# jeffpeterson/hypermerge

Hardware: AMD Instinct MI355X
Metric: merged changes/sec (1M docs×8 actors) at 1/2/4/8 GPUs + % HBM roofline (higher is better)
Workload: dtype u32; 1 GPU; C4: 1000000 docs/GPU x 8 actors x 64 changes/doc, map LWW sets; docs_per_gpu=1000000, changes_per_gpu=64000000, ops_per_gpu=96000538, parallelism=doc-shard1

## Files before the change

hypermerge_amd/csrc/merge_kernels.hip:

```cpp
#include <hip/hip_runtime.h>
#include <stdint.h>
#include "../../include/hypermerge_amd.h"
#include "merge_kernels.h"
#include "wave.h"

#ifndef HM_ABLATE
#define HM_ABLATE 0
#endif
#ifndef HM_STAMPS
#define HM_STAMPS 0
#endif
#define HM_NSTAMP 20
#ifndef HM_WAVES_PER_EU_OPL4
#define HM_WAVES_PER_EU_OPL4 3
#endif
#ifndef HM_WAVES_PER_EU_LIST3
#define HM_WAVES_PER_EU_LIST3 3
#endif
#ifndef HM_PRIO_PUSH
#define HM_PRIO_PUSH 2
#endif
#ifndef HM_PRIO_IO
#define HM_PRIO_IO 1
#endif
#ifndef HM_PRIO_HIST
#define HM_PRIO_HIST 3
#endif
#ifndef HM_PRIO_RANK
#define HM_PRIO_RANK 2
#endif
#ifndef HM_PRIO_K2
#define HM_PRIO_K2 2
#endif
#ifndef HM_PRIO_K1
#define HM_PRIO_K1 3
#endif
#ifndef HM_ASYNC_MAX_OPL
#define HM_ASYNC_MAX_OPL 2
#endif
#ifndef HM_ASYNC_STORES
#define HM_ASYNC_STORES 10
#endif
#ifndef HM_ASYNC_CHECK
#define HM_ASYNC_CHECK 0
#endif
#ifndef HM_WAVES_PER_EU
#define HM_WAVES_PER_EU 5
#endif
#ifndef HM_WAVES_PER_EU_WIDE
#define HM_WAVES_PER_EU_WIDE 4
#endif
#define WAVE 64
#define NA_MAX 8
#define NDEP_MAX 1024
typedef unsigned long long u64;
#if defined(__HIP_DEVICE_COMPILE__)
#define LDS __attribute__((address_space(3)))
#else
#define LDS
#endif

namespace hm {

__device__ __forceinline__ u64 readlane64(u64 v, int l) {
    const uint32_t lo = __builtin_amdgcn_readlane((int)(uint32_t)v, l);
    const uint32_t hi = __builtin_amdgcn_readlane((int)(uint32_t)(v >> 32), l);
    return ((u64)hi << 32) | lo;
}
__device__ __forceinline__ uint32_t shfl32(uint32_t v, int src) {
    return (uint32_t)__builtin_amdgcn_ds_bpermute(src << 2, (int)v);
}
__device__ __forceinline__ u64 shfl64(u64 v, int src) {
    return ((u64)shfl32((uint32_t)(v >> 32), src) << 32) | shfl32((uint32_t)v, src);
}
__device__ __forceinline__ u64 wave_or64(u64 v) {
    for (int o = 1; o < WAVE; o <<= 1) v |= shfl64(v, (int)(threadIdx.x ^ o));
    return v;
}
__device__ __forceinline__ uint32_t wave_excl_scan(uint32_t v, uint32_t *total) {
    uint32_t x = v;
    x += (uint32_t)__builtin_amdgcn_update_dpp(0, (int)x, DPP_ROW_SHR(1), 0xF, 0xF, false);
    x += (uint32_t)__builtin_amdgcn_update_dpp(0, (int)x, DPP_ROW_SHR(2), 0xF, 0xF, false);
    x += (uint32_t)__builtin_amdgcn_update_dpp(0, (int)x, DPP_ROW_SHR(4), 0xF, 0xF, false);
    x += (uint32_t)__builtin_amdgcn_update_dpp(0, (int)x, DPP_ROW_SHR(8), 0xF, 0xF, false);
    x += (uint32_t)__builtin_amdgcn_update_dpp(0, (int)x, DPP_ROW_BCAST15, 0xA, 0xF, false);
    x += (uint32_t)__builtin_amdgcn_update_dpp(0, (int)x, DPP_ROW_BCAST31, 0xC, 0xF, false);
    *total = (uint32_t)__builtin_amdgcn_readlane((int)x, WAVE - 1);
    return x - v;
}
__device__ __forceinline__ uint32_t wave_max(uint32_t v) {
    uint32_t x = v, y;
    y = (uint32_t)__builtin_amdgcn_update_dpp(0, (int)x, DPP_ROW_SHR(1), 0xF, 0xF, false); x = x > y ? x : y;
    y = (uint32_t)__builtin_amdgcn_update_dpp(0, (int)x, DPP_ROW_SHR(2), 0xF, 0xF, false); x = x > y ? x : y;
    y = (uint32_t)__builtin_amdgcn_update_dpp(0, (int)x, DPP_ROW_SHR(4), 0xF, 0xF, false); x = x > y ? x : y;
    y = (uint32_t)__builtin_amdgcn_update_dpp(0, (int)x, DPP_ROW_SHR(8), 0xF, 0xF, false); x = x > y ? x : y;
    y = (uint32_t)__builtin_amdgcn_update_dpp(0, (int)x, DPP_ROW_BCAST15, 0xA, 0xF, false); x = x > y ? x : y;
    y = (uint32_t)__builtin_amdgcn_update_dpp(0, (int)x, DPP_ROW_BCAST31, 0xC, 0xF, false); x = x > y ? x : y;
    return (uint32_t)__builtin_amdgcn_readlane((int)x, WAVE - 1);
}
__device__ __forceinline__ uint32_t bytesum64(u64 x) {
    return __builtin_amdgcn_sad_u8((uint32_t)x, 0u, __builtin_amdgcn_sad_u8((uint32_t)(x >> 32), 0u, 0u));
}
__device__ __forceinline__ uint32_t prev_lane(uint32_t v) {
    return (uint32_t)__builtin_amdgcn_update_dpp(0, (int)v, DPP_WAVE_SHR1, 0xF, 0xF, false);
}
__device__ __forceinline__ uint32_t fresh_lane() {
    uint32_t l;
    asm volatile("v_mov_b32 %0, %1" : "=v"(l) : "v"((uint32_t)threadIdx.x));
    return l;
}
template <bool FRESH> __device__ __forceinline__ uint32_t lane_id() {
    if constexpr (FRESH) return fresh_lane();
    else return threadIdx.x;
}
template <int OPL, bool LISTS, int CLS> struct Diet { static constexpr bool on = OPL <= 2 && !LISTS && CLS != 1; };
__device__ __forceinline__ void wave_sync() {
    __builtin_amdgcn_fence(__ATOMIC_SEQ_CST, "wavefront");
    __builtin_amdgcn_wave_barrier();
}

__device__ __forceinline__ u64 err_key(uint32_t h, uint32_t op_plus1, uint32_t arr, uint32_t code) {
    return ((u64)h << 40) | ((u64)(op_plus1 & 0xFFFF) << 24) | ((u64)(arr & 0xFFFF) << 8) | code;
}

struct SmallLds {
    LDS u64 *anc, *chain, *segor, *errkey, *cov;
    LDS u64 *opval;
    LDS u64 *survpk;
    LDS int64_t *survsum;
    LDS uint32_t *first, *base, *bclock, *headv, *objslot, *segcnt, *survcnt, *regoff, *regobj, *insmin;
    LDS uint32_t *flags, *deps, *depinfo;
    LDS uint8_t *seglist;
    LDS uint16_t *survp;
    LDS uint32_t *opro;
    LDS uint32_t *opmeta;
    LDS uint32_t *opelem;
    LDS int32_t *hist_of;
    LDS uint16_t *survop, *opbase;
    LDS uint16_t *oppar;
    LDS uint8_t *h2a, *chactor, *objtype;
    LDS uint16_t *opchg;
    LDS uint32_t *nins, *pcount, *nodekey, *tour0, *listbase;
    LDS uint16_t *poff;
    LDS uint16_t *nodeop, *nodepi, *regnode, *plist, *fc, *ns, *listid;
    LDS u64 *stamps;
};
#define PAR_HEAD 0xFFFFu
template <bool LISTS> struct Stride {
    static constexpr uint32_t reg = LISTS ? 1 : 4;
    static constexpr uint32_t seg = LISTS ? 1 : 2;
    static constexpr uint32_t op = LISTS ? 1 : 2;
};

template <int CLS> struct SizeClass;
template <> struct SizeClass<0> { static constexpr uint32_t NR = 32, NO = 16, ND = 128; };
template <> struct SizeClass<1> { static constexpr uint32_t NR = 256, NO = 64, ND = 512; };
template <> struct SizeClass<2> { static constexpr uint32_t NR = 128, NO = 32, ND = 256; };

template <typename L_t, typename P>
__host__ __device__ inline size_t small_carve(P base, uint32_t NOp, uint32_t NR, uint32_t NO, uint32_t ND,
                                              bool lists, bool counters, L_t *L) {
    size_t o = 0;
#define TAKE(f, T, cnt) do { L->f = (decltype(L->f))(base + o); o = (o + (size_t)(cnt) * sizeof(T) + 15) & ~(size_t)15; } while (0)
    TAKE(anc, u64, 64);          TAKE(chain, u64, NA_MAX);     TAKE(opval, u64, NOp);
    TAKE(errkey, u64, 1);        TAKE(base, uint32_t, NA_MAX * 3);
    if (lists) {
        TAKE(survcnt, uint32_t, NR); TAKE(regoff, uint32_t, NR);   TAKE(regobj, uint32_t, NR);
        TAKE(insmin, uint32_t, NR);  TAKE(flags, uint32_t, 2);
        TAKE(opmeta, uint32_t, NOp); TAKE(opro, uint32_t, NOp);
    } else {
        TAKE(survcnt, uint32_t, 4 * NR);                           TAKE(flags, uint32_t, 2);
        L->regoff = L->survcnt + 1; L->insmin = L->survcnt + 2;    L->regobj = L->survcnt + 3;
        TAKE(opro, uint32_t, 2 * NOp);
        L->opmeta = L->opro + 1;
    }
    TAKE(survop, uint16_t, NOp); TAKE(chactor, uint8_t, 64);   TAKE(objtype, uint8_t, NO);
    if (lists) {
        TAKE(opelem, uint32_t, NOp);
        L->nodekey = L->opelem;
        TAKE(nins, uint32_t, 1);
    }
    TAKE(stamps, u64, HM_STAMPS ? HM_NSTAMP + 1 : 0);
    const size_t dead_at = o;
    TAKE(hist_of, int32_t, 64);  TAKE(cov, u64, 1);            TAKE(opbase, uint16_t, 64);
    TAKE(oppar, uint16_t, lists ? NOp : 0);
    TAKE(h2a, uint8_t, 64);      TAKE(opchg, uint16_t, NOp);
    const size_t k1_at = o;
    TAKE(first, uint32_t, NA_MAX * 64);
    TAKE(deps, uint32_t, ND > NOp ? ND : NOp);
    TAKE(depinfo, uint32_t, ND);
    const size_t k1_end = o;
    o = k1_at;
    if (lists) { TAKE(segor, u64, NR);  TAKE(survpk, u64, NR); }
    else { TAKE(segor, u64, 2 * NR);    L->survpk = L->segor + 1; }
    TAKE(segcnt, uint32_t, NR);
    TAKE(objslot, uint32_t, NO);
    if (o < k1_end) o = k1_end;
    L->seglist = (decltype(L->seglist))L->first; L->survp = (decltype(L->survp))L->first;
    if (lists) {
        const uint32_t NP = NR + NO, NE = 2 * (NOp + NO);
        size_t q = dead_at;
#define TAKEK(f, T, cnt) do { L->f = (decltype(L->f))(base + q); q = (q + (size_t)(cnt) * sizeof(T) + 15) & ~(size_t)15; } while (0)
        TAKEK(tour0, uint32_t, NE);     TAKEK(pcount, uint32_t, NP);  TAKEK(listbase, uint32_t, NO + 1);
        TAKEK(poff, uint16_t, NP + 1);  TAKEK(survp, uint16_t, NOp);
        TAKEK(nodeop, uint16_t, NOp);   TAKEK(nodepi, uint16_t, NOp); TAKEK(regnode, uint16_t, NR);
        TAKEK(plist, uint16_t, NOp);    TAKEK(fc, uint16_t, NP);      TAKEK(ns, uint16_t, NOp);
        TAKEK(listid, uint16_t, NO);    TAKEK(seglist, uint8_t, NOp);
#undef TAKEK
        if (q > o) o = q;
    }
    TAKE(survsum, int64_t, counters ? NOp : 0);
#undef TAKE
    L->bclock = L->base + NA_MAX;
    L->headv = L->base + 2 * NA_MAX;
    return o;
}

template <typename T> struct Id { typedef T type; };
template <typename T> __device__ __forceinline__ T lds_or(LDS T *p, typename Id<T>::type v) { return __atomic_fetch_or(p, v, __ATOMIC_RELAXED); }
template <typename T> __device__ __forceinline__ T lds_min(LDS T *p, typename Id<T>::type v) { return __atomic_fetch_min(p, v, __ATOMIC_RELAXED); }
template <typename T> __device__ __forceinline__ T lds_max(LDS T *p, typename Id<T>::type v) { return __atomic_fetch_max(p, v, __ATOMIC_RELAXED); }
template <typename T> __device__ __forceinline__ T lds_add(LDS T *p, typename Id<T>::type v) { return __atomic_fetch_add(p, v, __ATOMIC_RELAXED); }

#if HM_STAMPS
__device__ unsigned long long hm_stamp_acc[HM_NSTAMP];
__device__ __forceinline__ u64 stamp_now() {
    u64 t;
    __builtin_amdgcn_sched_barrier(0);
    asm volatile("s_memtime %0\n\ts_waitcnt lgkmcnt(0)" : "=s"(t) :: "memory");
    __builtin_amdgcn_sched_barrier(0);
    return t;
}
#define STAMP(L_, i) do { const u64 t_ = stamp_now(); if (threadIdx.x == 0) { (L_).stamps[i] += t_ - (L_).stamps[HM_NSTAMP]; (L_).stamps[HM_NSTAMP] = t_; } } while (0)
#elif defined(HM_MARKS)
#define STAMP(L_, i) asm volatile(";HMMARK " #i)
#else
#define STAMP(L_, i) do { } while (0)
#endif

enum : uint32_t { FL_UNSUPPORTED = 1u };
enum Outcome { OUT_OK = 0, OUT_ERROR = 1, OUT_UNSUPPORTED = 2, OUT_INVALID = 3 };

__device__ __forceinline__ void need_set(uint32_t &lo, uint32_t &hi, uint32_t a, uint32_t v) {
    const uint32_t sh = (a & 3) * 8;
    const uint32_t w = a < 4 ? lo : hi;
    const uint32_t cur = (w >> sh) & 0xFF;
    const uint32_t nw = v > cur ? ((w & ~(0xFFu << sh)) | (v << sh)) : w;
    lo = a < 4 ? nw : lo;
    hi = a < 4 ? hi : nw;
}


__device__ __forceinline__ uint32_t fidx(uint32_t a, uint32_t s) { return (s & 63) * NA_MAX + (a & (NA_MAX - 1)); }
__device__ __forceinline__ void clear_first(LDS uint32_t *first, uint32_t lane) {
    static_assert(NA_MAX * 64 == 2 * WAVE * 4, "first-table size");
    LDS uint4 *f4 = (LDS uint4 *)first;
    const uint4 ones = make_uint4(~0u, ~0u, ~0u, ~0u);
    f4[lane] = ones;
    f4[lane + WAVE] = ones;
}

__device__ __forceinline__ uint32_t tie_order(uint32_t pc) { return (pc & 1) ? (0x10000u - pc) : (0x20000u + pc); }


template <int OPL>
__device__ __forceinline__ void rga_order(const SmallLds &L, uint32_t R, uint32_t O,
                                          const uint32_t (&oreg)[OPL], const uint32_t (&oobj)[OPL],
                                          const uint32_t (&opar)[OPL], const uint32_t (&oact)[OPL],
                                          const uint32_t (&oelem)[OPL], const uint32_t (&oarr)[OPL],
                                          const int32_t (&oh)[OPL], uint32_t *epos) {
    const uint32_t lane = threadIdx.x;
    const uint32_t NP = R + O;
    constexpr uint32_t END = 0xFFFFu;
    for (uint32_t i = lane; i < NP; i += WAVE) { L.pcount[i] = 0; L.fc[i] = 0xFFFFu; }
    for (uint32_t i = lane; i < R; i += WAVE) L.regnode[i] = 0xFFFFu;
    if (lane == 0) *L.nins = 0;
    uint32_t nl = 0;
    for (uint32_t o0 = 0; o0 < O; o0 += WAVE) {
        const uint32_t o = o0 + lane;
// ... 317 lines not shown
        if (lane < n) f(lane);
        if constexpr (CAP > WAVE) { if (lane + WAVE < n) f(lane + WAVE); }
    } else {
        for (uint32_t i = lane; i < n; i += WAVE) f(i);
    }
}
template <int OPL, bool LISTS, bool DIET, typename C>
__device__ __forceinline__ void stage_rows(const SmallParams &p, const SmallLds &L, const hm_doc_row &doc, const Rows &r) {
    const uint32_t lane = lane_id<DIET>(), m = doc.n_ops;
    stage_op<LISTS>(L, lane, m, r.a0, r.b0);
    if (OPL > 1) stage_op<LISTS>(L, lane + WAVE, m, r.a1, r.b1);
    if (OPL > 2) stage_op<LISTS>(L, lane + 2 * WAVE, m, r.a2, r.b2);
    if (OPL > 3) stage_op<LISTS>(L, lane + 3 * WAVE, m, r.a3, r.b3);
    const uint32_t nd = doc.n_deps < C::ND ? doc.n_deps : C::ND;
    if (lane < nd) L.deps[lane] = pack_dep(r.d0);
    if (lane + WAVE < nd) L.deps[lane + WAVE] = pack_dep(r.d1);
    if constexpr (C::ND > 2 * WAVE)
        for (uint32_t i = lane + 2 * WAVE; i < nd; i += WAVE)
            L.deps[i] = pack_dep(*reinterpret_cast<const uint2 *>(p.deps + doc.dep_off + i));
}
__device__ __forceinline__ hm_change_row change_of(uint2 w0, uint2 w1, uint2 w2) {
    hm_change_row c;
    c.actor = (uint16_t)(w0.x & 0xFFFF); c.n_deps = (uint16_t)(w0.x >> 16); c.seq = w0.y;
    c.dep_off = w1.x; c.n_ops = w1.y; c.op_first = w2.x; c.content_id = w2.y;
    return c;
}
struct DocState {
    int32_t hist;
    uint32_t H, total;
    bool doc_lists;
    bool counters;
};

struct OpCheck { uint32_t err; bool surv, has_list, late; };
template <bool LISTS>
__device__ __forceinline__ OpCheck op_check(const SmallLds &L, int32_t ohv, uint32_t act, uint32_t obj, uint32_t reg,
                                            uint32_t par, uint32_t okey, uint32_t R, uint32_t O) {
    const bool asg = ohv >= 0 && act >= HM_INS && act <= HM_INC && reg < R;
    const uint32_t oi = obj < O ? obj : 0u, ri = reg < R ? reg : 0u;
    const uint32_t os = obj < O ? L.objslot[oi] : 0xFFFFFFFFu;
    const uint32_t pi = par < R ? par : 0u;
    uint32_t ot = 0, im = 0, ip = 0;
    if constexpr (LISTS) { ot = L.objtype[oi]; im = L.insmin[ri]; ip = L.insmin[pi]; }
    const u64 so = L.segor[Stride<LISTS>::seg * ri];
    const uint32_t h = ohv < 0 ? 0u : (uint32_t)ohv;
    const bool unknown = asg && (os == 0xFFFFFFFFu || os > okey);
    const bool known = asg && !unknown;
    if constexpr (!LISTS) {
        OpCheck r;
        r.has_list = false; r.late = false;
        r.surv = known && (act == HM_SET || act == HM_LINK) && !((so >> h) & 1);
        r.err = unknown ? (uint32_t)HM_ERR_UNKNOWN_OBJECT : 0u;
        return r;
    }
    const bool is_list = ot == HM_MAKE_LIST || ot == HM_MAKE_TEXT;
    const bool ins = known && act == HM_INS;
    const bool sl = known && (act == HM_SET || act == HM_LINK);
    OpCheck r;
    r.has_list = ins || (known && is_list);
    r.surv = sl && !((so >> h) & 1);
    r.late = ins && par != HM_HEAD && !(ip <= okey);
    uint32_t e = 0;
    if (sl && is_list && !(im <= okey)) e = HM_ERR_MISSING_ELEM;
    if (ins && im != okey + 1) e = HM_ERR_DUPLICATE_ELEM;
    if (unknown) e = HM_ERR_UNKNOWN_OBJECT;
    r.err = e;
    return r;
}

template <int OPL, bool LISTS, bool DIET, typename C>
__device__ __forceinline__ Outcome merge_doc_small(const SmallParams &p, const SmallLds &L, const hm_doc_row &doc,
                                                   const uint2 w0, const uint2 w1, const uint2 w2, DocState &st) {
    uint32_t lane = lane_id<DIET>();
    constexpr uint32_t RS = Stride<LISTS>::reg, SS = Stride<LISTS>::seg, OS = Stride<LISTS>::op;
    const uint32_t n = doc.n_changes, A = doc.n_actors, m = doc.n_ops, R = doc.n_regs, O = doc.n_objs;
    st.hist = -1; st.H = 0; st.total = 0; st.doc_lists = false; st.counters = false;

    if (HM_ABLATE & 8) return OUT_UNSUPPORTED;
    STAMP(L, 0);
    if (HM_PRIO_K1) __builtin_amdgcn_s_setprio(HM_PRIO_K1);
    const bool act = lane < n;
    const hm_change_row c = change_of(w0, w1, w2);
    clear_first(L.first, lane);
    if (lane < NA_MAX) { L.base[lane] = 0xFFFFFFFFu; L.bclock[lane] = 0; L.headv[lane] = 0; L.chain[lane] = 0; }
    if (lane == 0) { *L.errkey = ~0ull; L.flags[0] = 0; L.flags[1] = 0; *L.cov = 0; }
    const uint32_t dep_lo = doc.dep_off, ndep = doc.n_deps;
    wave_sync();
    const uint32_t actor = c.actor, seq = c.seq;
    const uint32_t my_dep0 = c.dep_off - dep_lo;
    const uint32_t op_end = c.op_first + c.n_ops, dep_end = c.dep_off + c.n_deps;
    const uint32_t prev_op = prev_lane(op_end), prev_dep = prev_lane(dep_end);
    bool bad = (n == 0 && (m || ndep)) ||
               (act && (c.op_first != (lane ? prev_op : doc.op_off) || c.dep_off != (lane ? prev_dep : dep_lo) ||
                        (lane == n - 1 && (op_end != doc.op_off + m || dep_end != dep_lo + ndep))));
    const bool rowok = act && !(actor >= A || seq == 0 || c.dep_off < dep_lo || my_dep0 + c.n_deps > ndep);
    bad |= act && !rowok;
    bad |= act && (c.op_first < doc.op_off || c.op_first - doc.op_off + c.n_ops > m);
    const uint32_t a8 = actor & (NA_MAX - 1);
    lds_min(&L.base[a8], rowok ? seq : 0xFFFFFFFFu);
    lds_max(&L.bclock[a8], rowok ? seq : 0u);
    L.chactor[lane] = (uint8_t)actor;
    L.opbase[lane] = (uint16_t)(c.op_first - doc.op_off);
    if (__ballot(bad)) return OUT_UNSUPPORTED;
    wave_sync();
    const uint32_t mybase = act ? L.base[a8] : 0;
    const uint32_t slot = seq - mybase;
    if (__ballot(act && slot >= 64)) return OUT_UNSUPPORTED;
    lds_min(&L.first[fidx(a8, (slot & 63))], act ? lane : 0xFFFFFFFFu);
    {
        const uint32_t o0 = c.op_first - doc.op_off;
        if (act) for (uint32_t j = 0; j < c.n_ops; j++) L.opchg[o0 + j] = (uint16_t)(lane | (a8 << 8));
    }
    wave_sync();

    STAMP(L, 1);
    if constexpr (DIET) lane = fresh_lane();
    if (HM_ABLATE & 16) return OUT_UNSUPPORTED;
    {
        bool bad_dep = false;
        for_rows<C::ND, LISTS>(lane, ndep, [&](uint32_t i) {
            const uint32_t pk = L.deps[i];
            const uint32_t a = pk >> 24, s = pk & 0xFFFFFF;
            bad_dep |= pk == 0xFFFFFFFFu || a >= A;
            const uint32_t ad = a & (NA_MAX - 1);
            const uint32_t b = L.base[ad];
            const bool inwin = b != 0xFFFFFFFFu && s >= b && s - b < 64;
            const uint32_t f = L.first[fidx(ad, ((s - b) & 63))];
            const uint32_t rel = s == 0 ? 0u : (inwin ? s - b + 1 : 0x7Fu);
            L.depinfo[i] = (inwin && f < 64 ? f : 0x7Fu) | (rel << 8) | (ad << 16);
        });
        if (__ballot(bad_dep)) return OUT_UNSUPPORTED;
    }
    const uint32_t first_me = act ? L.first[fidx(actor, slot)] : lane;
    const bool dup = act && first_me != lane;
    const uint32_t cid_first = shfl32(c.content_id, (int)(first_me & 63));
    u64 dmask = 0;
    uint32_t pred_arr = 0xFFu;
    bool ok = true;
    bool own_row = false;
    wave_sync();
    {
        const uint32_t maxd = wave_max(act ? (uint32_t)c.n_deps : 0u);
        for (uint32_t j0 = 0; j0 < maxd; j0 += 2) {
            uint32_t inf[2];
#pragma unroll
            for (int u = 0; u < 2; u++) {
                const bool live = act && j0 + u < c.n_deps;
                inf[u] = L.depinfo[live ? my_dep0 + j0 + u : 0u];
            }
#pragma unroll
            for (int u = 0; u < 2; u++) {
                const bool live = act && j0 + u < c.n_deps;
                const uint32_t a = (inf[u] >> 16) & (NA_MAX - 1), rel = (inf[u] >> 8) & 0x7F, f = inf[u] & 0x7F;
                own_row |= live && a == actor;
                const bool use = live && a != actor && rel != 0;
                ok = ok && !(use && (rel == 0x7F || f >= lane));
                dmask |= (use && rel != 0x7F && f < lane) ? (1ull << f) : 0ull;
            }
        }
        const uint32_t ps = seq - 1;
        const bool hp = act && ps != 0, inb = ps >= mybase;
        const uint32_t f = L.first[fidx(a8, ((ps - mybase) & 63))];
        ok = ok && !(hp && (!inb || f >= lane));
        const bool pv = hp && inb && f < lane;
        dmask |= pv ? (1ull << (f & 63)) : 0ull;
        pred_arr = pv ? f : pred_arr;
        ok = ok && !(dup && cid_first != c.content_id);
// ... 325 lines not shown
    }
    if (hv) { lds_or(L.cov, D); lds_or(&L.chain[hactor], 1ull << lane); }
    uint32_t alo = hv && lane < 32 ? 1u << lane : 0u, ahi = hv && lane >= 32 ? 1u << (lane - 32) : 0u;
    if (HM_ABLATE & 1024) return OUT_UNSUPPORTED;
    {
        if (HM_PRIO_PUSH) __builtin_amdgcn_s_setprio(HM_PRIO_PUSH);
        const uint32_t Hs = (uint32_t)__builtin_amdgcn_readfirstlane((int)H);
        const uint32_t Dlo = (uint32_t)D, Dhi = (uint32_t)(D >> 32);
        const uint32_t H1 = Hs < 32 ? Hs : 32;
#define PUSH_BC(v, k) ((uint32_t)__builtin_amdgcn_readlane((int)(v), (int)(k)))
#define PUSH_LO(k) alo |= PUSH_BC(alo, (k)) & (uint32_t)__builtin_amdgcn_sbfe((int)Dlo, (k), 1)
#define PUSH_HI(k) do { const uint32_t m_ = (uint32_t)__builtin_amdgcn_sbfe((int)Dhi, (k) - 32, 1);          \
                        const uint32_t bl_ = PUSH_BC(alo, (k)), bh_ = PUSH_BC(ahi, (k));                   \
                        alo |= bl_ & m_; ahi |= bh_ & m_; } while (0)
#pragma unroll
        for (int g = 0; g < 32; g += 8) {
            if ((uint32_t)g >= H1) break;
            PUSH_LO(g); PUSH_LO(g + 1); PUSH_LO(g + 2); PUSH_LO(g + 3);
            PUSH_LO(g + 4); PUSH_LO(g + 5); PUSH_LO(g + 6); PUSH_LO(g + 7);
        }
#pragma unroll
        for (int g = 32; g < 64; g += 8) {
            if ((uint32_t)g >= Hs) break;
            PUSH_HI(g); PUSH_HI(g + 1); PUSH_HI(g + 2); PUSH_HI(g + 3);
            PUSH_HI(g + 4); PUSH_HI(g + 5); PUSH_HI(g + 6); PUSH_HI(g + 7);
        }
#undef PUSH_LO
#undef PUSH_HI
#undef PUSH_BC
        if (HM_PRIO_PUSH) __builtin_amdgcn_s_setprio(0);
    }
    const u64 anc = hv ? ((((u64)ahi << 32) | alo) & ~(1ull << lane)) : 0ull;
    if (hv) L.anc[lane] = anc;
    wave_sync();
    STAMP(L, 4);
    if constexpr (DIET) lane = fresh_lane();
    if (HM_ABLATE & 64) return OUT_UNSUPPORTED;
    const u64 covered = *L.cov;
    bool suspect = false;
    if constexpr (LISTS) {
        if (hv && (Dnp & (Dnp - 1))) {
            u64 x = Dnp;
            while (x) {
                const uint32_t i2 = (uint32_t)__builtin_ctzll(x);
                x &= x - 1;
                if (L.anc[i2] & Dnp) suspect = true;
            }
        }
    } else {
        const u64 rest = Dnp & (Dnp - 1);
        const bool two = hv && rest != 0;
        if (__ballot(two)) {
            const u64 a1 = L.anc[two ? (uint32_t)__builtin_ctzll(rest) : 0u];
            u64 x = two ? rest & (rest - 1) : 0ull;
            suspect = two && (a1 & Dnp) != 0;
            if (__ballot(x != 0)) {
                while (x) {
                    const uint32_t i2 = (uint32_t)__builtin_ctzll(x);
                    x &= x - 1;
                    if (L.anc[i2] & Dnp) suspect = true;
                }
            }
        }
    }
    uint32_t h_own_row = own_row ? 1u : 0u, h_dep0 = my_dep0, h_nd = c.n_deps;
    if (!identity) {
        h_own_row = shfl32(h_own_row, (int)ai); h_dep0 = shfl32(my_dep0, (int)ai); h_nd = shfl32(c.n_deps, (int)ai);
    }
    suspect |= hv && h_own_row != 0;
    if (suspect) {
        const FoldView fv = {L.anc, L.chain, L.first, L.base, L.deps, L.hist_of};
        if (fold_differs(fv, h_dep0, h_nd, hactor, hseq)) lds_or(L.flags, FL_UNSUPPORTED);
    }
    if (hv && !((covered >> lane) & 1)) L.headv[hactor] = hseq;
    for_rows<C::NO, LISTS>(lane, O, [&](uint32_t i) {
        L.objslot[i] = i == 0 ? 0u : 0xFFFFFFFFu;
        if constexpr (LISTS) L.objtype[i] = i == 0 ? HM_MAKE_MAP : 0xFF;
    });
    for_rows<C::NR, LISTS>(lane, R, [&](uint32_t i) {
        if constexpr (LISTS) {
            L.segor[i] = 0; L.segcnt[i] = 0; L.survpk[i] = 0; L.insmin[i] = 0xFFFFFFFFu; L.regobj[i] = HM_NONE;
        } else {
            static_assert(Stride<false>::reg == 4 && Stride<false>::seg == 2, "row widths");
            *(LDS uint4 *)(L.survcnt + 4 * i) = make_uint4(0u, 0u, 0xFFFFFFFFu, HM_NONE);
            *(LDS uint4 *)(L.segor + 2 * i) = make_uint4(0u, 0u, 0u, 0u);
            L.segcnt[i] = 0;
        }
    });
    wave_sync();

    STAMP(L, 5);
    if constexpr (DIET) lane = fresh_lane();
    if (HM_PRIO_K2) __builtin_amdgcn_s_setprio(HM_PRIO_K2);
    if (HM_ABLATE & 2) return OUT_UNSUPPORTED;
    uint32_t oreg[OPL], oobj[OPL], opar[OPL], oact[OPL], okey[OPL], oarr[OPL], oelem[OPL], oactor[OPL];
    int32_t oh[OPL];
    bool counter_ops = false, malformed = false;
    if constexpr (!LISTS) {
        uint2 ow[OPL];
        uint32_t cw[OPL], ob[OPL];
        int32_t hr[OPL];
        u64 an[OPL];
#pragma unroll
        for (int t = 0; t < OPL; t++) { ow[t] = *(LDS uint2 *)(L.opro + 2 * (lane + WAVE * t)); cw[t] = L.opchg[lane + WAVE * t]; }
#pragma unroll
        for (int t = 0; t < OPL; t++) {
            const uint32_t ch = lane + WAVE * t < m ? cw[t] & 0xFFu : 0u;
            oarr[t] = ch; oactor[t] = (cw[t] >> 8) & (NA_MAX - 1);
            ob[t] = L.opbase[ch];
            hr[t] = identity ? (int32_t)ch : L.hist_of[ch];
        }
#pragma unroll
        for (int t = 0; t < OPL; t++) {
            oh[t] = lane + WAVE * t < m ? hr[t] : -1;
            an[t] = L.anc[oh[t] < 0 ? 0 : oh[t]];
        }
        bool listy = false;
#pragma unroll
        for (int t = 0; t < OPL; t++) {
            const uint32_t k = lane + WAVE * t;
            const bool live = k < m, applied = oh[t] >= 0;
            const uint32_t a = live ? ow[t].y & 0xFF : 0xFFu;
            oact[t] = a; oreg[t] = ow[t].x & 0xFFFFu; oobj[t] = ow[t].x >> 16; opar[t] = 0; oelem[t] = 0;
            okey[t] = ((uint32_t)(applied ? oh[t] : 0) << 16) | (k - ob[t]);
            counter_ops |= live & ((a == HM_INC) | (((ow[t].y >> 8) & 0xFF) == HM_DT_COUNTER));
            const bool make = a <= HM_MAKE_TEXT;
            const bool bad = live & (make ? oobj[t] >= O : ((a > HM_INC) | (oreg[t] >= R)));
            malformed |= bad;
            listy |= (a == HM_INS) | (applied & ((a == HM_MAKE_LIST) | (a == HM_MAKE_TEXT)));
            const bool asg = applied & !bad & !make & (a != HM_INS) & (oobj[t] < O);
            if (applied & !bad & make) lds_min(&L.objslot[oobj[t]], okey[t] + 1);
            if (asg) { L.regobj[4 * oreg[t]] = oobj[t]; lds_add(&L.segcnt[oreg[t]], 1u); }
            if (asg && a != HM_INC) lds_or(&L.segor[2 * oreg[t]], an[t]);
        }
        malformed |= listy;
    } else {
#pragma unroll
    for (int t = 0; t < OPL; t++) {
        const uint32_t k = lane + WAVE * t;
        oh[t] = -1; okey[t] = 0; oarr[t] = 0; oreg[t] = 0; oobj[t] = 0; opar[t] = 0; oact[t] = 0xFF; oelem[t] = 0; oactor[t] = 0;
        if (k < m) {
            const uint32_t meta = L.opmeta[k], ro = L.opro[k], pr = L.oppar[k];
            const uint32_t cw = L.opchg[k], ch = cw & 0xFFu;
            oarr[t] = ch; oactor[t] = cw >> 8; oh[t] = identity ? (int32_t)ch : L.hist_of[ch];
            oreg[t] = ro & 0xFFFFu; oobj[t] = ro >> 16; oact[t] = meta & 0xFF;
            opar[t] = pr == PAR_HEAD ? HM_HEAD : pr;
            if (LISTS) {
                oelem[t] = L.opelem[k];
                if (oact[t] == HM_INS && oelem[t] >= (1u << 24)) lds_or(L.flags, FL_UNSUPPORTED);
            }
            counter_ops |= oact[t] == HM_INC || ((meta >> 8) & 0xFF) == HM_DT_COUNTER;
            okey[t] = ((uint32_t)(oh[t] < 0 ? 0 : oh[t]) << 16) | (k - L.opbase[ch]);
            const uint32_t a = oact[t];
            const bool bad = a <= HM_MAKE_TEXT ? oobj[t] >= O
                           : (a <= HM_INC ? (oreg[t] >= R || (a == HM_INS && opar[t] != HM_HEAD && opar[t] >= R)) : true);
            malformed |= bad;
            if (oh[t] >= 0 && !bad) {
                if (a <= HM_MAKE_TEXT) lds_min(&L.objslot[oobj[t]], okey[t] + 1);
                else if (oobj[t] < O) {
                    L.regobj[oreg[t]] = oobj[t];
                    if (a == HM_INS) lds_min(&L.insmin[oreg[t]], okey[t] + 1);
                    else {
                        lds_add(&L.segcnt[oreg[t]], 1u);
                        if (a != HM_INC) lds_or(&L.segor[oreg[t]], L.anc[oh[t]]);
                    }
                }
            }
        }
// ... 51 lines not shown
    if constexpr (DIET) lane = fresh_lane();
    if (HM_PRIO_K2 && !HM_PRIO_RANK) __builtin_amdgcn_s_setprio(0);
    if (HM_PRIO_RANK) __builtin_amdgcn_s_setprio(HM_PRIO_RANK);
    if (HM_ABLATE & 4) return OUT_UNSUPPORTED;
    uint32_t total = 0;
    const uint32_t lane_s = LISTS ? lane : fresh_lane();
    auto offsets = [&](uint32_t r) {
        uint32_t tot;
        const uint32_t cnt = r < R ? bytesum64(L.survpk[SS * r]) : 0u;
        const uint32_t ex = wave_excl_scan(cnt, &tot);
        if constexpr (LISTS) { if (r < R) { L.regoff[r] = total + ex; L.survcnt[r] = cnt; } }
        else if (r < R) *(LDS uint2 *)(L.survcnt + 4 * r) = make_uint2(cnt, total + ex);
        total += tot;
    };
    if constexpr (C::NR <= 2 * WAVE && !LISTS) {
        offsets(lane_s);
        if constexpr (C::NR > WAVE) { if (R > WAVE) offsets(lane_s + WAVE); }
    } else {
        for (uint32_t r0 = 0; r0 < R; r0 += WAVE) offsets(r0 + lane_s);
    }
    wave_sync();
    uint32_t my_act[OPL], rb0[OPL], rank[OPL];
    bool tie[OPL];
#pragma unroll
    for (int t = 0; t < OPL; t++) {
        const uint32_t ri = surv[t] ? oreg[t] : 0u;
        my_act[t] = surv[t] ? oactor[t] : 0u;
        rb0[t] = L.regoff[RS * ri];
        const u64 pk = L.survpk[SS * ri];
        const uint32_t sh = 8 * (my_act[t] + 1);
        rank[t] = surv[t] ? bytesum64(sh >= 64 ? 0ull : pk >> sh) : 0u;
        tie[t] = surv[t] && ((pk >> (8 * my_act[t])) & 0xFF) > 1;
    }
    bool anytie = false;
#pragma unroll
    for (int t = 0; t < OPL; t++) anytie |= tie[t];
    if (__ballot(anytie)) {
        uint32_t myt[OPL];
        bool oddn[OPL];
#pragma unroll
        for (int t = 0; t < OPL; t++) {
            myt[t] = 0;
            oddn[t] = tie[t] && (L.segcnt[tie[t] ? oreg[t] : 0u] & 1);
            u64 tm = __ballot(tie[t]);
            while (tm) {
                const int j = (int)__builtin_ctzll(tm);
                tm &= tm - 1;
                const uint32_t rj = (uint32_t)__builtin_amdgcn_readlane((int)oreg[t], j);
                const uint32_t kj = (uint32_t)__builtin_amdgcn_readlane((int)okey[t], j);
                uint32_t pc = 0;
#pragma unroll
                for (int t2 = 0; t2 < OPL; t2++)
                    pc += (uint32_t)__popcll(__ballot(oh[t2] >= 0 && oact[t2] >= HM_SET && oact[t2] <= HM_INC &&
                                                      oreg[t2] == rj && okey[t2] < kj));
                if ((int)lane == j) myt[t] = tie_order(pc);
            }
        }
#pragma unroll
        for (int t = 0; t < OPL; t++) {
            u64 tm = __ballot(tie[t]);
            while (tm) {
                const int j = (int)__builtin_ctzll(tm);
                tm &= tm - 1;
                const uint32_t rj = (uint32_t)__builtin_amdgcn_readlane((int)oreg[t], j);
                const uint32_t aj = (uint32_t)__builtin_amdgcn_readlane((int)my_act[t], j);
                const uint32_t tj = (uint32_t)__builtin_amdgcn_readlane((int)myt[t], j);
#pragma unroll
                for (int t2 = 0; t2 < OPL; t2++) {
                    const bool peer = tie[t2] && oreg[t2] == rj && my_act[t2] == aj && !(t2 == t && (int)lane == j);
                    rank[t2] += (peer && (oddn[t2] ? (tj > myt[t2]) : (tj < myt[t2]))) ? 1u : 0u;
                }
            }
        }
    }
#pragma unroll
    for (int t = 0; t < OPL; t++) {
        if (!surv[t]) continue;
        const uint32_t pos = rb0[t] + rank[t];
        uint32_t tag = 0;
        if (LISTS ? p.counters != 0 : doc_counters) {
            const uint32_t mt = L.opmeta[OS * (lane + WAVE * t)], vt = (mt >> 16) & 0xFF;
            const bool cset = (mt & 0xFF) == HM_SET && ((mt >> 8) & 0xFF) == HM_DT_COUNTER && (vt == HM_V_INT || vt == HM_V_FLOAT);
            tag = cset ? (0x8000u | (vt == HM_V_INT ? 0x4000u : 0u) | ((uint32_t)oh[t] << 8)) : 0u;
            L.survsum[pos] = 0;
        }
        L.survop[pos] = (uint16_t)((lane + WAVE * t) | tag);
    }
    wave_sync();
    if (HM_PRIO_RANK) __builtin_amdgcn_s_setprio(0);
    STAMP(L, 8);
    if constexpr (DIET) lane = fresh_lane();
    if (HM_ABLATE & 256) return OUT_UNSUPPORTED;
    if constexpr (LISTS) {
        if (doc_lists)
            rga_order<OPL>(L, R, O, oreg, oobj, opar, oact, oelem, oarr, oh, p.res_epos ? p.res_epos + doc.reg_off : nullptr);
    }
    if (LISTS ? (p.counters && __ballot(counter_ops)) : doc_counters) {
        bool outside = false;
        int64_t incv[OPL];
        u64 basev[OPL];
#pragma unroll
        for (int t = 0; t < OPL; t++) {
            incv[t] = (oh[t] >= 0 && oact[t] == HM_INC) ? (int64_t)op_value(L, lane + WAVE * t) : 0;
            const uint32_t q = lane + WAVE * t;
            basev[t] = 0;
            if (q < total) {
                const uint32_t sw = L.survop[q];
                if ((sw & 0xC000u) == 0xC000u) basev[t] = op_value(L, sw & 0xFFu);
            }
        }
#pragma unroll
        for (int t = 0; t < OPL; t++) {
            if (oh[t] < 0 || oact[t] != HM_INC) continue;
            const uint32_t k = lane + WAVE * t;
            const uint32_t reg = oreg[t], b0 = L.regoff[RS * reg], cnt = L.survcnt[RS * reg];
            const u64 an = L.anc[oh[t]];
            const uint32_t my_vtag = (L.opmeta[OS * k] >> 16) & 0xFF;
            const int64_t v = incv[t];
            for (uint32_t q = 0; q < cnt; q++) {
                const uint32_t sw = L.survop[b0 + q];
                if (!(sw & 0x8000u)) continue;
                if (!((an >> ((sw >> 8) & 63u)) & 1)) continue;
                if (!(sw & 0x4000u) || my_vtag != HM_V_INT || (u64)(v < 0 ? -v : v) >= (1ull << 44)) { outside = true; continue; }
                lds_add((LDS u64 *)&L.survsum[b0 + q], (unsigned long long)v);
            }
        }
#pragma unroll
        for (int t = 0; t < OPL; t++) {
            const int64_t b = (int64_t)basev[t];
            outside |= (u64)(b < 0 ? -b : b) >= (1ull << 52);
        }
        if (__ballot(outside)) return OUT_UNSUPPORTED;
        wave_sync();
    }
    st.hist = hist; st.H = H; st.total = total; st.doc_lists = doc_lists; st.counters = doc_counters;
    return OUT_OK;
}

__device__ __forceinline__ uint32_t min_cmp_of(const SmallParams &p, const SmallLds &L, const hm_doc_row &doc, uint32_t mc,
                                               uint32_t lane) {
    const uint32_t S = p.a_stride;
    const uint32_t bc = (lane < S && lane < doc.n_actors) ? L.bclock[lane] : 0u;
    const bool aGTE = __ballot(lane < S && bc < mc) == 0;
    const bool bGTE = __ballot(lane < S && mc < bc) == 0;
    return p.min_clock ? ((aGTE && bGTE) ? 0u : (aGTE ? 1u : (bGTE ? 2u : 3u))) : 0u;
}

template <int OPL> struct SurvRows { hm_surv_result r[OPL]; };
template <int OPL, bool LISTS>
__device__ __forceinline__ SurvRows<OPL> surv_rows(const SmallParams &p, const SmallLds &L, const DocState &st, uint32_t lane) {
    SurvRows<OPL> o;
#pragma unroll
    for (int t = 0; t < OPL; t++) {
        const uint32_t q = lane + WAVE * t;
        const uint32_t k = q < st.total ? (L.survop[q] & 0xFFu) : 0u, mt = L.opmeta[Stride<LISTS>::op * k];
        hm_surv_result sr;
        sr.op = k; sr.vtag = (mt >> 16) & 0xFF; sr.value = op_value(L, k);
        if ((LISTS ? p.counters != 0 : st.counters) && q < st.total && (mt & 0xFF) == HM_SET && ((mt >> 8) & 0xFF) == HM_DT_COUNTER && sr.vtag == HM_V_INT)
            sr.value = (u64)((int64_t)sr.value + L.survsum[q]);
        o.r[t] = sr;
    }
    return o;
}

__device__ __forceinline__ void st16(void *dst, uint4 v) { *reinterpret_cast<uint4 *>(dst) = v; }
__device__ __forceinline__ void st4(void *dst, uint32_t v) { *reinterpret_cast<uint32_t *>(dst) = v; }
__device__ __forceinline__ void put_status_row(hm_doc_result *dres, uint32_t status, uint32_t err_change, uint32_t err_op) {
// ... 28 lines not shown
        for (uint32_t a = lane; a < S; a += WAVE) { ck[a] = 0u; hd[a] = 0u; bk[a] = 0u; }
        return;
    }
    if (oc == OUT_UNSUPPORTED) {
        if (lane == 0) {
            put_status_row(dres_of(), (uint32_t)HM_DEFERRED, HM_NONE, HM_NONE);
#if !HM_ABLATE
            p.deferred[atomicAdd(p.n_deferred, 1u)] = d;
#endif
        }
        return;
    }
    if constexpr (DIET)
        asm volatile("" :: "s"(p.res_docs), "s"(p.res_clock), "s"(p.res_back_clock), "s"(p.res_heads), "s"(p.res_hist),
                     "s"(p.res_all_deps), "s"(p.res_regs), "s"(p.res_surv));
    hm_reg_result *regs = p.res_regs + doc.reg_off;
    for_rows<C::NR, LISTS>(lane, R, [&](uint32_t r) {
        if constexpr (LISTS) {
            const int32_t li = st.doc_lists ? (int32_t)L.insmin[r] : -1;
            st16(regs + r, make_uint4(L.survcnt[r], L.regoff[r], (uint32_t)li, L.regobj[r]));
        } else {
            static_assert(sizeof(hm_reg_result) == 16 && Stride<false>::reg == 4, "register rows are stored whole");
            st16(reinterpret_cast<char *>(regs) + r * 16u, *(LDS uint4 *)(L.survcnt + 4 * r));
        }
    });
    if (lane < n) {
        const u64 an = st.hist >= 0 ? L.anc[st.hist] : 0ull;
        uint32_t *row = (p.res_all_deps + (size_t)doc.change_off * S) + lane * S;
        if (S == 8 || S == 4) {
            uint32_t v[NA_MAX];
#pragma unroll
            for (int a = 0; a < NA_MAX; a++) v[a] = (uint32_t)__popcll(an & L.chain[a]);
            st16(row, make_uint4(v[0], v[1], v[2], v[3]));
            if (S == 8) st16(row + 4, make_uint4(v[4], v[5], v[6], v[7]));
        } else {
            for (uint32_t a = 0; a < S; a++) row[a] = a < NA_MAX ? (uint32_t)__popcll(an & L.chain[a]) : 0u;
        }
    }
    uint32_t *ck = p.res_clock + (size_t)ds * S, *hd = p.res_heads + (size_t)ds * S, *bk = p.res_back_clock + (size_t)ds * S;
    if (lane < S) {
        const bool ar = lane < A;
        ck[lane] = ar ? (uint32_t)__popcll(L.chain[lane]) : 0u;
        hd[lane] = ar ? L.headv[lane] : 0u;
        bk[lane] = ar ? L.bclock[lane] : 0u;
    }
    for (uint32_t a = WAVE + lane; a < S; a += WAVE) { ck[a] = 0u; hd[a] = 0u; bk[a] = 0u; }
    const bool act = lane < n;
    const u64 q = __ballot(act && st.hist == -1);
    if (act) st4((p.res_hist + doc.change_off) + lane, (uint32_t)st.hist);
    if (lane == 0) {
        hm_doc_result r = {};
        r.status = HM_OK; r.err_change = HM_NONE; r.err_op = HM_NONE;
        r.hist_len = st.H; r.n_queued = (uint32_t)__popcll(q); r.n_surv = st.total;
        r.min_cmp = mcmp;
        *dres_of() = r;
    }
#pragma unroll
    for (int t = 0; t < OPL; t++) {
        const uint32_t q = lane + WAVE * t;
        if (q < st.total) st16((p.res_surv + doc.op_off) + q, make_uint4(sv.r[t].op, sv.r[t].vtag, (uint32_t)sv.r[t].value,
                                                                       (uint32_t)(sv.r[t].value >> 32)));
    }
}

template <int OPL>
__device__ __forceinline__ uint32_t out_stores_min(const SmallParams &p, const hm_doc_row &doc, const DocState &st) {
    const uint32_t S = p.a_stride, n = doc.n_changes;
    uint32_t c = (doc.n_regs + WAVE - 1) / WAVE;
    if (n) c += (S == 8 ? 2u : 1u) + 1u;
    c += 3u + 2u;
    c += (st.total + WAVE - 1) / WAVE < (uint32_t)OPL ? (st.total + WAVE - 1) / WAVE : (uint32_t)OPL;
    return c;
}
template <int OPL>
__device__ __forceinline__ void pad_stores(const SmallParams &p, const hm_doc_row &doc, const DocState &st, uint32_t ds, bool ok) {
    uint32_t *pad = &p.res_docs[ds].pad;
    const uint32_t zero = 0u;
    for (uint32_t c = ok ? out_stores_min<OPL>(p, doc, st) : 0u; c < HM_ASYNC_STORES; c++)
        asm volatile("global_store_dword %0, %1, off" :: "v"(pad), "v"(zero) : "memory");
}

template <int OPL, bool LISTS, int CLS>
__global__ __launch_bounds__(WAVE) __attribute__((amdgpu_waves_per_eu(OPL >= 3 ? (LISTS ? (OPL == 3 ? HM_WAVES_PER_EU_LIST3 : HM_WAVES_PER_EU_OPL4 - 1) : HM_WAVES_PER_EU_OPL4)
                                              : (!LISTS && CLS != 1 ? HM_WAVES_PER_EU : HM_WAVES_PER_EU_WIDE))))
void merge_small_kernel(SmallParams p) {
    extern __shared__ __align__(16) uint8_t lds_raw[];
    typedef SizeClass<CLS> C;
    constexpr bool DIET = Diet<OPL, LISTS, CLS>::on;
    SmallLds L;
    small_carve((LDS uint8_t *)lds_raw, WAVE * OPL, C::NR, C::NO, C::ND, LISTS, true, &L);
    p.cap_regs = C::NR; p.cap_objs = C::NO; p.cap_deps = C::ND;
    typedef __attribute__((address_space(4))) const SmallParams KParams;
    KParams *kp = (KParams *)__builtin_amdgcn_kernarg_segment_ptr();
    uint32_t d = blockIdx.x;
    if (p.xcd_remap && (gridDim.x & 7) == 0) d = (blockIdx.x & 7) * (gridDim.x >> 3) + (blockIdx.x >> 3);
    if (d >= p.n_docs) return;
#if HM_STAMPS
    if (threadIdx.x == 0) { for (int i = 0; i < HM_NSTAMP; i++) L.stamps[i] = 0; L.stamps[HM_NSTAMP] = stamp_now(); }
#endif
    hm_doc_row doc = p.docs[d];
    bool dok = check_doc(p, doc);
    uint2 w0, w1, w2;
    {
        const Rows r = load_rows<OPL>(p, doc);
        stage_rows<OPL, LISTS, DIET, C>(p, L, doc, r);
        w0 = make_uint2(r.c01.x, r.c01.y); w1 = make_uint2(r.c01.z, r.c01.w); w2 = r.c2;
    }
    wave_sync();
    for (;;) {
        asm volatile("" : "+s"(kp));
        const SmallParams &p = *(const SmallParams *)kp;
        if constexpr (DIET)
            asm volatile("" :: "s"(p.n_docs), "s"(p.a_stride), "s"(p.general_only), "s"(p.docs), "s"(p.min_clock), "s"(p.doc_slot));
        const uint32_t dn = d + gridDim.x;
        const bool more = dn < p.n_docs;
        bool dokn = true;
        hm_doc_row docn = {};
        static_assert(sizeof(hm_doc_row) == 12 * sizeof(uint32_t), "doc row words");
        const uint32_t lane0 = lane_id<DIET>();
        uint32_t docw = 0;
        if (more && lane0 < 12) docw = reinterpret_cast<const uint32_t *>(p.docs + dn)[lane0];
        auto take_docn = [&]() {
            uint32_t w[12];
#pragma unroll
            for (int j = 0; j < 12; j++) w[j] = (uint32_t)__builtin_amdgcn_readlane((int)docw, j);
            __builtin_memcpy(&docn, w, sizeof docn);
        };
        Rows next;
        AsyncRows anext;
        constexpr bool ASY = OPL <= HM_ASYNC_MAX_OPL;
        const bool in_env = doc.n_changes <= 64 && doc.n_actors <= NA_MAX && doc.n_ops <= WAVE * OPL && doc.n_ops < 256 &&
                            doc.n_regs <= C::NR && doc.n_objs <= C::NO && doc.n_objs >= 1 &&
                            doc.n_deps <= C::ND && !p.general_only;
        DocState st;
        const uint32_t ds = hm_slot(p, d);
        uint32_t mc = 0;
        if (p.min_clock && lane0 < p.a_stride) mc = (p.min_clock + (size_t)ds * p.a_stride)[lane0];
        if (p.min_clock && p.a_stride > WAVE) {
            uint32_t extra = 0;
            for (uint32_t a = WAVE + threadIdx.x; a < p.a_stride; a += WAVE) extra |= p.min_clock[(size_t)ds * p.a_stride + a];
            if (__ballot(extra != 0) && threadIdx.x == NA_MAX) mc |= 1u;
        }
        const Outcome oc = !dok ? OUT_INVALID : in_env ? merge_doc_small<OPL, LISTS, DIET, C>(p, L, doc, w0, w1, w2, st) : OUT_UNSUPPORTED;
        STAMP(L, 9);
        const uint32_t lane_io = lane_id<DIET>();
        uint32_t mcmp = oc == OUT_OK ? min_cmp_of(p, L, doc, mc, lane_io) : 0u;
        asm volatile("" : "+s"(mcmp) :: "memory");
        asm volatile("" : "+v"(docw));
        if (more) {
            if constexpr (DIET)
                asm volatile("" :: "s"(p.changes), "s"(p.deps), "s"(p.ops), "s"(p.a_stride), "s"(p.lim_changes), "s"(p.lim_deps),
                             "s"(p.lim_ops), "s"(p.lim_regs));
            take_docn();
            dokn = check_doc(p, docn);
            if constexpr (ASY) anext = load_rows_async<OPL, LISTS>(p, docn, lane_io);
            else next = load_rows<OPL>(p, docn);
        }
        STAMP(L, 12);
        if (HM_PRIO_IO) __builtin_amdgcn_s_setprio(HM_PRIO_IO);
        const SurvRows<OPL> sv = surv_rows<OPL, LISTS>(p, L, st, lane_io);
        write_outputs<OPL, LISTS, DIET, C>(p, L, d, ds, doc, oc, st, mcmp, sv, lane_io);
        if constexpr (ASY) { if (more) pad_stores<OPL>(p, doc, st, ds, oc == OUT_OK); }
        wave_sync();
        STAMP(L, 10);
        if (!more) break;
        if constexpr (ASY) {
            next = take_rows_async<OPL, DIET>(anext, docn);
// ... 24 lines not shown
    const uint32_t x = v ? a[(size_t)row * S + col] : 0, y = v ? b[(size_t)row * S + col] : 0;
    const u64 lt = __ballot(v && x < y), gt = __ballot(v && y < x);
    if (v && col == 0) {
        const u64 mask = (S >= 64 ? ~0ull : ((1ull << S) - 1)) << lane;
        const bool aGTE = (lt & mask) == 0, bGTE = (gt & mask) == 0;
        out[row] = (aGTE && bGTE) ? 0 : (aGTE ? 1 : (bGTE ? 2 : 3));
    }
}
__global__ void clock_union_kernel(const uint32_t *a, const uint32_t *b, uint32_t *c, size_t n) {
    for (size_t i = blockIdx.x * (size_t)blockDim.x + threadIdx.x; i < n; i += (size_t)gridDim.x * blockDim.x)
        c[i] = a[i] > b[i] ? a[i] : b[i];
}
__global__ void clock_intersection_kernel(const uint32_t *a, const uint32_t *b, uint32_t *c, size_t n) {
    for (size_t i = blockIdx.x * (size_t)blockDim.x + threadIdx.x; i < n; i += (size_t)gridDim.x * blockDim.x)
        c[i] = a[i] < b[i] ? a[i] : b[i];
}

}

extern "C" int hm_debug_async_check(unsigned long long *out2, int reset) {
#if HM_ASYNC_CHECK
    if (!out2 || hipDeviceSynchronize() != hipSuccess) return -1;
    if (hipMemcpyFromSymbol(&out2[0], HIP_SYMBOL(hm::hm_async_checked), 8) != hipSuccess ||
        hipMemcpyFromSymbol(&out2[1], HIP_SYMBOL(hm::hm_async_bad), 8) != hipSuccess) return -1;
    if (reset) {
        const unsigned long long z = 0;
        if (hipMemcpyToSymbol(HIP_SYMBOL(hm::hm_async_checked), &z, 8) != hipSuccess ||
            hipMemcpyToSymbol(HIP_SYMBOL(hm::hm_async_bad), &z, 8) != hipSuccess) return -1;
    }
    return 1;
#else
    (void)out2; (void)reset;
    return 0;
#endif
}
#if HM_STAMPS
extern "C" int hm_debug_stamps(unsigned long long *out, int n, int reset) {
    if (n > HM_NSTAMP) n = HM_NSTAMP;
    if (hipDeviceSynchronize() != hipSuccess) return -1;
    if (hipMemcpyFromSymbol(out, HIP_SYMBOL(hm::hm_stamp_acc), n * sizeof(unsigned long long)) != hipSuccess) return -1;
    if (reset) {
        unsigned long long z[HM_NSTAMP] = {};
        if (hipMemcpyToSymbol(HIP_SYMBOL(hm::hm_stamp_acc), z, sizeof z) != hipSuccess) return -1;
    }
    return n;
}
#endif
uint32_t hm_small_class(uint32_t max_regs, uint32_t max_objs, uint32_t max_deps) {
    typedef hm::SizeClass<0> S0;
    typedef hm::SizeClass<2> S2;
    if (max_regs <= S0::NR && max_objs <= S0::NO && max_deps <= S0::ND) return 0u;
    if (max_regs <= S2::NR && max_objs <= S2::NO && max_deps <= S2::ND) return 2u;
    return 1u;
}

template <int CLS> static size_t carve_of(uint32_t opl, bool lists, bool counters) {
    hm::SmallLds L;
    typedef hm::SizeClass<CLS> C;
    return hm::small_carve((uintptr_t)0, 64 * opl, C::NR, C::NO, C::ND, lists, counters, &L);
}

size_t hm_small_lds_bytes(uint32_t opl, uint32_t cls, bool lists, bool counters) {
    return cls == 0 ? carve_of<0>(opl, lists, counters) : cls == 2 ? carve_of<2>(opl, lists, counters) : carve_of<1>(opl, lists, counters);
}

typedef void (*SmallKernel)(SmallParams);
template <bool LISTS, int CLS> static SmallKernel small_kernel_opl(uint32_t opl) {
    switch (opl) {
    case 1: return hm::merge_small_kernel<1, LISTS, CLS>;
    case 2: return hm::merge_small_kernel<2, LISTS, CLS>;
    case 3: return hm::merge_small_kernel<3, LISTS, CLS>;
    default: return hm::merge_small_kernel<4, LISTS, CLS>;
    }
}
static SmallKernel hm_small_kernel(uint32_t opl, uint32_t cls, bool lists) {
    if (cls == 0) return lists ? small_kernel_opl<true, 0>(opl) : small_kernel_opl<false, 0>(opl);
    if (cls == 2) return lists ? small_kernel_opl<true, 2>(opl) : small_kernel_opl<false, 2>(opl);
    return lists ? small_kernel_opl<true, 1>(opl) : small_kernel_opl<false, 1>(opl);
}

uint32_t hm_small_occupancy(uint32_t opl, uint32_t cls, bool lists, bool counters) {
    const size_t lds = hm_small_lds_bytes(opl, cls, lists, counters);
    int n = 0;
    const int by_lds = (int)(160u * 1024u / ((lds + 511) & ~(size_t)511));
    (void)hipOccupancyMaxActiveBlocksPerMultiprocessor(&n, hm_small_kernel(opl, cls, lists), WAVE, lds);
    if (n > by_lds) n = by_lds;
    return n > 0 ? (uint32_t)n : 1u;
}

hipError_t hm_launch_small(const SmallParams &p, uint32_t opl, uint32_t cls, bool lists, uint32_t grid, hipStream_t s) {
    const size_t lds = hm_small_lds_bytes(opl, cls, lists, p.counters != 0);
    hipLaunchKernelGGL(hm_small_kernel(opl, cls, lists), dim3(grid), dim3(WAVE), lds, s, p);
    return hipGetLastError();
}

hipError_t hm_launch_clock(int which, const uint32_t *a, const uint32_t *b, void *out, uint32_t n_docs,
                           uint32_t S, hipStream_t s) {
    if (which == 0) {
        if (S == 0 || S > HM_MAX_STRIDE) return hipErrorInvalidValue;
        const uint32_t rows_per_wave = 64 / S;
        const uint32_t waves = (n_docs + rows_per_wave - 1) / rows_per_wave;
        const uint32_t blocks = (waves + 3) / 4;
        hipLaunchKernelGGL(hm::clock_cmp_kernel, dim3(blocks ? blocks : 1), dim3(256), 0, s, a, b, (uint8_t *)out, n_docs, S);
    } else {
        const size_t n = (size_t)n_docs * S;
        uint32_t blocks = (uint32_t)((n + 255) / 256);
        if (blocks > 8192) blocks = 8192;
        if (which == 1) hipLaunchKernelGGL(hm::clock_union_kernel, dim3(blocks ? blocks : 1), dim3(256), 0, s, a, b, (uint32_t *)out, n);
        else hipLaunchKernelGGL(hm::clock_intersection_kernel, dim3(blocks ? blocks : 1), dim3(256), 0, s, a, b, (uint32_t *)out, n);
    }
    return hipGetLastError();
}
```

Measured before the change: 35.06 billion changes/s.

## Shrink small-kernel LDS footprint by aliasing non-list rows into K1 scratch

For map-only docs with at most two ops per lane, the survcnt/survop rows move into the region reused after the first phase, and depinfo is aliased onto the anc buffer. This cuts per-block LDS so more blocks can be resident per CU. The change also makes zero constants opaque in DIET kernels to limit SGPR/VGPR materialization, adds a separate waves-per-EU knob for size class 2, and makes the occupancy estimate use 1280-byte LDS granularity. Aliasing risks lifetime overlap bugs if survcnt or depinfo are touched while the first-phase or anc data is still live.

Result: no change. 34.92 billion changes/s, median of 3 (-0.4%).

```diff
diff --git a/hypermerge_amd/csrc/merge_kernels.hip b/hypermerge_amd/csrc/merge_kernels.hip
--- a/hypermerge_amd/csrc/merge_kernels.hip
+++ b/hypermerge_amd/csrc/merge_kernels.hip
@@ -46,6 +46,9 @@
 #endif
 #ifndef HM_WAVES_PER_EU
 #define HM_WAVES_PER_EU 5
+#endif
+#ifndef HM_WAVES_PER_EU_CLS2
+#define HM_WAVES_PER_EU_CLS2 5
 #endif
 #ifndef HM_WAVES_PER_EU_WIDE
 #define HM_WAVES_PER_EU_WIDE 4
@@ -112,6 +115,11 @@
 template <bool FRESH> __device__ __forceinline__ uint32_t lane_id() {
     if constexpr (FRESH) return fresh_lane();
     else return threadIdx.x;
+}
+template <bool FRESH> __device__ __forceinline__ u64 zero64() {
+    uint32_t z = 0u;
+    if constexpr (FRESH) asm volatile("" : "+v"(z));
+    return ((u64)z << 32) | z;
 }
 template <int OPL, bool LISTS, int CLS> struct Diet { static constexpr bool on = OPL <= 2 && !LISTS && CLS != 1; };
 __device__ __forceinline__ void wave_sync() {
@@ -161,6 +169,7 @@
 __host__ __device__ inline size_t small_carve(P base, uint32_t NOp, uint32_t NR, uint32_t NO, uint32_t ND,
                                               bool lists, bool counters, L_t *L) {
     size_t o = 0;
+    const bool k1_rows = !lists && NOp <= 2 * WAVE;
 #define TAKE(f, T, cnt) do { L->f = (decltype(L->f))(base + o); o = (o + (size_t)(cnt) * sizeof(T) + 15) & ~(size_t)15; } while (0)
     TAKE(anc, u64, 64);          TAKE(chain, u64, NA_MAX);     TAKE(opval, u64, NOp);
     TAKE(errkey, u64, 1);        TAKE(base, uint32_t, NA_MAX * 3);
@@ -169,12 +178,13 @@
         TAKE(insmin, uint32_t, NR);  TAKE(flags, uint32_t, 2);
         TAKE(opmeta, uint32_t, NOp); TAKE(opro, uint32_t, NOp);
     } else {
-        TAKE(survcnt, uint32_t, 4 * NR);                           TAKE(flags, uint32_t, 2);
-        L->regoff = L->survcnt + 1; L->insmin = L->survcnt + 2;    L->regobj = L->survcnt + 3;
+        if (!k1_rows) TAKE(survcnt, uint32_t, 4 * NR);
+        TAKE(flags, uint32_t, 2);
         TAKE(opro, uint32_t, 2 * NOp);
         L->opmeta = L->opro + 1;
     }
-    TAKE(survop, uint16_t, NOp); TAKE(chactor, uint8_t, 64);   TAKE(objtype, uint8_t, NO);
+    if (!k1_rows) TAKE(survop, uint16_t, NOp);
+    TAKE(chactor, uint8_t, 64);  TAKE(objtype, uint8_t, NO);
     if (lists) {
         TAKE(opelem, uint32_t, NOp);
         L->nodekey = L->opelem;
@@ -188,13 +198,19 @@
     const size_t k1_at = o;
     TAKE(first, uint32_t, NA_MAX * 64);
     TAKE(deps, uint32_t, ND > NOp ? ND : NOp);
-    TAKE(depinfo, uint32_t, ND);
+    if (k1_rows && ND * sizeof(uint32_t) <= 64 * sizeof(u64)) L->depinfo = (decltype(L->depinfo))L->anc;
+    else TAKE(depinfo, uint32_t, ND);
     const size_t k1_end = o;
     o = k1_at;
     if (lists) { TAKE(segor, u64, NR);  TAKE(survpk, u64, NR); }
     else { TAKE(segor, u64, 2 * NR);    L->survpk = L->segor + 1; }
     TAKE(segcnt, uint32_t, NR);
     TAKE(objslot, uint32_t, NO);
+    if (k1_rows) {
+        TAKE(survcnt, uint32_t, 4 * NR);
+        TAKE(survop, uint16_t, NOp);
+    }
+    if (!lists) { L->regoff = L->survcnt + 1; L->insmin = L->survcnt + 2; L->regobj = L->survcnt + 3; }
     if (o < k1_end) o = k1_end;
     L->seglist = (decltype(L->seglist))L->first; L->survp = (decltype(L->survp))L->first;
     if (lists) {
@@ -678,7 +694,7 @@
     const bool act = lane < n;
     const hm_change_row c = change_of(w0, w1, w2);
     clear_first(L.first, lane);
-    if (lane < NA_MAX) { L.base[lane] = 0xFFFFFFFFu; L.bclock[lane] = 0; L.headv[lane] = 0; L.chain[lane] = 0; }
+    if (lane < NA_MAX) { L.base[lane] = 0xFFFFFFFFu; L.bclock[lane] = 0; L.headv[lane] = 0; L.chain[lane] = zero64<DIET>(); }
     if (lane == 0) { *L.errkey = ~0ull; L.flags[0] = 0; L.flags[1] = 0; *L.cov = 0; }
     const uint32_t dep_lo = doc.dep_off, ndep = doc.n_deps;
     wave_sync();
@@ -1170,8 +1186,10 @@
             L.segor[i] = 0; L.segcnt[i] = 0; L.survpk[i] = 0; L.insmin[i] = 0xFFFFFFFFu; L.regobj[i] = HM_NONE;
         } else {
             static_assert(Stride<false>::reg == 4 && Stride<false>::seg == 2, "row widths");
-            *(LDS uint4 *)(L.survcnt + 4 * i) = make_uint4(0u, 0u, 0xFFFFFFFFu, HM_NONE);
-            *(LDS uint4 *)(L.segor + 2 * i) = make_uint4(0u, 0u, 0u, 0u);
+            uint32_t zero = 0u, ones = 0xFFFFFFFFu, none = HM_NONE;
+            if constexpr (DIET) asm volatile("" : "+v"(zero), "+v"(ones), "+v"(none));
+            *(LDS uint4 *)(L.survcnt + 4 * i) = make_uint4(zero, zero, ones, none);
+            *(LDS uint4 *)(L.segor + 2 * i) = make_uint4(zero, zero, zero, zero);
             L.segcnt[i] = 0;
         }
     });
@@ -1389,7 +1407,7 @@
             const uint32_t mt = L.opmeta[OS * (lane + WAVE * t)], vt = (mt >> 16) & 0xFF;
             const bool cset = (mt & 0xFF) == HM_SET && ((mt >> 8) & 0xFF) == HM_DT_COUNTER && (vt == HM_V_INT || vt == HM_V_FLOAT);
             tag = cset ? (0x8000u | (vt == HM_V_INT ? 0x4000u : 0u) | ((uint32_t)oh[t] << 8)) : 0u;
-            L.survsum[pos] = 0;
+            L.survsum[pos] = (int64_t)zero64<DIET>();
         }
         L.survop[pos] = (uint16_t)((lane + WAVE * t) | tag);
     }
@@ -1584,7 +1602,7 @@
 
 template <int OPL, bool LISTS, int CLS>
 __global__ __launch_bounds__(WAVE) __attribute__((amdgpu_waves_per_eu(OPL >= 3 ? (LISTS ? (OPL == 3 ? HM_WAVES_PER_EU_LIST3 : HM_WAVES_PER_EU_OPL4 - 1) : HM_WAVES_PER_EU_OPL4)
-                                              : (!LISTS && CLS != 1 ? HM_WAVES_PER_EU : HM_WAVES_PER_EU_WIDE))))
+                                              : (!LISTS && CLS != 1 ? (CLS == 0 ? HM_WAVES_PER_EU : HM_WAVES_PER_EU_CLS2) : HM_WAVES_PER_EU_WIDE))))
 void merge_small_kernel(SmallParams p) {
     extern __shared__ __align__(16) uint8_t lds_raw[];
     typedef SizeClass<CLS> C;
@@ -1775,9 +1793,12 @@
 uint32_t hm_small_occupancy(uint32_t opl, uint32_t cls, bool lists, bool counters) {
     const size_t lds = hm_small_lds_bytes(opl, cls, lists, counters);
     int n = 0;
-    const int by_lds = (int)(160u * 1024u / ((lds + 511) & ~(size_t)511));
+    const int by_lds = (int)(160u * 1024u / ((lds + 1279) / 1280 * 1280));
     (void)hipOccupancyMaxActiveBlocksPerMultiprocessor(&n, hm_small_kernel(opl, cls, lists), WAVE, lds);
     if (n > by_lds) n = by_lds;
+#ifdef HM_FORCE_PER_CU
+    if (opl <= 2 && cls == 0 && !lists) n = HM_FORCE_PER_CU;
+#endif
     return n > 0 ? (uint32_t)n : 1u;
 }
 
```
